# BattleZips/BattleZips-Halo2

Measured on AMD Instinct MI355X. Metric: complete proofs per second (synthesis + create_proof), BoardCircuit, k=14, IPA/Pasta, higher is better.
Workload: dtype u32x8 (255-bit modular integer, Montgomery)

## Files before the change

battlezips-halo2_amd/bzh2/__init__.py:

```python
from __future__ import annotations

import ctypes
import os

import numpy as np

_PKG = os.path.dirname(os.path.abspath(__file__))
_LIB_PATH = os.path.join(os.path.dirname(_PKG), "libbzh2.so")

OK, E_ARG, E_OOM, E_HIP, E_RANGE, E_NOGPU = 0, -1, -2, -3, -4, -5
CURVE_VESTA, CURVE_PALLAS, CURVE_BN254 = 0, 1, 2
FIELD_FP, FIELD_FQ, FIELD_BN254_FR, FIELD_BN254_FQ = 0, 1, 2, 3
FORM_CANONICAL, FORM_MONTGOMERY = 0, 1
MEM_HOST, MEM_DEVICE = 0, 1
T_MSM_DIGITS, T_MSM_ACCUMULATE, T_MSM_REDUCE, T_MSM_FINALIZE, T_NTT, T_COUNT = 0, 1, 2, 3, 4, 8
TIMER_NAMES = {0: "msm_digits", 1: "msm_accumulate", 2: "msm_reduce", 3: "msm_finalize", 4: "ntt"}

CURVE_SCALAR_FIELD = {CURVE_VESTA: FIELD_FP, CURVE_PALLAS: FIELD_FQ, CURVE_BN254: FIELD_BN254_FR}

EXPORTS = [
    "bzh_version", "bzh_strerror", "bzh_device_count", "bzh_ctx_create", "bzh_ctx_create_on_stream",
    "bzh_ctx_destroy", "bzh_ctx_sync", "bzh_last_error", "bzh_ctx_profile", "bzh_ctx_timings", "bzh_ctx_work", "bzh_ctx_msm_additions",
    "bzh_bases_upload", "bzh_bases_precompute", "bzh_bases_free", "bzh_bases_len", "bzh_bases_walk", "bzh_bases_points", "bzh_msm", "bzh_ntt", "bzh_coeff_to_extended",
    "bzh_jacobian_to_affine", "bzh_jacobian_sum", "bzh_affine_compress", "bzh_field_omega",
]


class BzhError(RuntimeError):
    def __init__(self, status: int, where: str, detail: str = ""):
        self.status = status
        super().__init__("%s failed: %s (%d)%s" % (where, _strerror(status), status, (": " + detail) if detail else ""))


_lib = None


def lib_path() -> str:
    return _LIB_PATH
# ... 16 lines not shown
    L.bzh_ctx_create_on_stream.argtypes = [ctypes.c_int, vp, ctypes.POINTER(vp)]
    L.bzh_ctx_destroy.argtypes = [vp]
    L.bzh_ctx_sync.argtypes = [vp]
    L.bzh_last_error.argtypes = [vp]
    L.bzh_last_error.restype = ctypes.c_char_p
    L.bzh_ctx_profile.argtypes = [vp, ctypes.c_int]
    L.bzh_ctx_timings.argtypes = [vp, ctypes.POINTER(ctypes.c_double), u64p]
    L.bzh_bases_upload.argtypes = [vp, ctypes.c_int, vp, ctypes.c_size_t, ctypes.c_int, ctypes.c_int, ctypes.POINTER(vp)]
    L.bzh_bases_precompute.argtypes = [vp, vp, ctypes.c_int]
    L.bzh_bases_free.argtypes = [vp, vp]
    L.bzh_bases_len.argtypes = [vp]
    L.bzh_bases_len.restype = ctypes.c_size_t
    L.bzh_msm.argtypes = [vp, vp, vp, ctypes.c_size_t, ctypes.c_size_t, ctypes.c_int, ctypes.c_int, vp]
    L.bzh_ntt.argtypes = [vp, ctypes.c_int, vp, ctypes.c_uint, ctypes.c_size_t, u64p, u64p, ctypes.c_int, ctypes.c_int,
                          ctypes.c_int]
    L.bzh_jacobian_to_affine.argtypes = [ctypes.c_int, u64p, ctypes.c_size_t, ctypes.c_int, u64p]
    L.bzh_affine_compress.argtypes = [ctypes.c_int, u64p, ctypes.c_size_t, ctypes.c_int, ctypes.POINTER(ctypes.c_uint8)]
    L.bzh_field_omega.argtypes = [ctypes.c_int, ctypes.c_uint, ctypes.c_int, u64p]
    _lib = L
    return L


def _strerror(status: int) -> str:
    try:
        return load().bzh_strerror(status).decode()
    except Exception:
        return "status %d" % status


def device_count() -> int:
# ... 130 lines not shown
            coset_shift: int | None = None, form: int = FORM_CANONICAL) -> np.ndarray:
        a = np.ascontiguousarray(data, dtype=np.uint64).copy()
        shape = a.shape
        if a.ndim == 2:
            a = a.reshape(1, *a.shape)
        batch, n = a.shape[0], a.shape[1]
        log_n = n.bit_length() - 1
        if n == 0 or (1 << log_n) != n:
            raise BzhError(E_ARG, "bzh_ntt", "length must be a power of two")
        w = field_omega(field, log_n, form) if omega is None else int_to_limbs(omega)
        cs = None if coset_shift is None else int_to_limbs(coset_shift)
        rc = load().bzh_ntt(self.handle, field, ctypes.c_void_p(a.ctypes.data), log_n, batch, _u64(w),
                            _u64(cs) if cs is not None else None, int(inverse), form, MEM_HOST)
        self._check(rc, "bzh_ntt")
        return a.reshape(shape)

    def coeff_to_extended(self, field: int, coeffs: np.ndarray, log_ext: int, omega_ext: int | None = None,
                          coset_shift: int | None = None, form: int = FORM_CANONICAL) -> np.ndarray:
        a = np.ascontiguousarray(coeffs, dtype=np.uint64)
        squeeze = a.ndim == 2
        if squeeze:
            a = a.reshape(1, *a.shape)
        batch, n = a.shape[0], a.shape[1]
        log_n = n.bit_length() - 1
        if n != 1 << log_n:
            raise BzhError(E_ARG, "bzh_coeff_to_extended", "length must be a power of two")
        w = field_omega(field, log_ext, form) if omega_ext is None else int_to_limbs(omega_ext)
        sh = None if coset_shift is None else int_to_limbs(coset_shift)
        out = np.zeros((batch, 1 << log_ext, 4), dtype=np.uint64)
        L = load()
# ... 353 lines not shown
```

battlezips-halo2_amd/csrc/capi.hip:

```cpp
#include <cstring>
#include <algorithm>
#include <thread>
#include <new>
#include <vector>

#include "ctx.hpp"
#include "curve.cuh"
#include "host_field.hpp"

namespace bzh {
void ntt_cache_drop(bzh_ctx* ctx);
}

using namespace bzh;

static bool valid_curve(int c) { return c >= 0 && c <= 2; }
static bool valid_field(int f) { return f >= 0 && f <= 3; }
static bool valid_form(int f) { return f == BZH_FORM_CANONICAL || f == BZH_FORM_MONTGOMERY; }
static bool valid_mem(int m) { return m == BZH_MEM_HOST || m == BZH_MEM_DEVICE; }
static unsigned field_two_adicity(int f) {
    unsigned s = 0;
    with_field(f, [&](auto p) {
        s = FieldInfo<decltype(p)>::S;
        return BZH_OK;
// ... 379 lines not shown
            const uint64_t* coset_shift, int inverse, int form, int mem) {
    if (!ctx || !data || !omega || !valid_field(field) || !valid_form(form) || !valid_mem(mem)) return BZH_E_ARG;
    if (log_n > field_two_adicity(field) || log_n > 30) return BZH_E_RANGE;
    if (batch == 0) return BZH_OK;
    std::lock_guard<std::mutex> lk(ctx->mu);
    BZH_HIP_TRY(ctx, hipSetDevice(ctx->device));
    if (mem == BZH_MEM_DEVICE) return ntt_run(ctx, field, (uint32_t*)data, log_n, batch, omega, coset_shift, inverse, form);
    void* stage = nullptr;
    const size_t bytes = (batch << log_n) * 32;
    int rc = ws_ensure(ctx, 3, bytes, &stage);
    if (rc) return rc;
    BZH_HIP_TRY(ctx, hipMemcpyAsync(stage, data, bytes, hipMemcpyHostToDevice, ctx->stream));
    rc = ntt_run(ctx, field, (uint32_t*)stage, log_n, batch, omega, coset_shift, inverse, form);
    if (rc) return rc;
    BZH_HIP_TRY(ctx, hipMemcpyAsync(data, stage, bytes, hipMemcpyDeviceToHost, ctx->stream));
    BZH_HIP_TRY(ctx, hipStreamSynchronize(ctx->stream));
    return BZH_OK;
}

int bzh_coeff_to_extended(bzh_ctx* ctx, int field, const uint64_t* coeffs, unsigned log_n, uint64_t* out, unsigned log_ext,
                          size_t batch, const uint64_t* omega_ext, const uint64_t* coset_shift, int form, int mem) {
    if (!ctx || !coeffs || !out || !omega_ext || !valid_field(field) || !valid_form(form) || !valid_mem(mem)) return BZH_E_ARG;
    if (log_ext > field_two_adicity(field) || log_ext > 30 || log_n > log_ext) return BZH_E_RANGE;
    if (batch == 0) return BZH_OK;
    std::lock_guard<std::mutex> lk(ctx->mu);
    BZH_HIP_TRY(ctx, hipSetDevice(ctx->device));
    const size_t in_elems = batch << log_n, out_elems = batch << log_ext;
    const uint32_t* d_in = (const uint32_t*)coeffs;
    uint32_t* d_out = (uint32_t*)out;
    void* stage = nullptr;
// ... 377 lines not shown
```

battlezips-halo2_amd/csrc/ctx.hpp:

```cpp
#pragma once
#include <hip/hip_runtime.h>
#include <sched.h>

#include <algorithm>
#include <cstdint>
#include <cstdlib>
#include <cstring>
#include <mutex>
#include <string>
#include <vector>

#include "../../include/bzh2.h"

struct bzh_bases {
    int curve = 0;
    size_t n = 0;
    uint32_t* d_xy = nullptr;
    int device = 0;
    int pre_c = 0;
    int pre_nwin = 0;
    size_t row_stride = 0;
    size_t vec_col_stride = 0;
    uint32_t* d_xy29 = nullptr;
};
// ... 213 lines not shown
            hipEvent_t e = ctx->event_pool.back();
            ctx->event_pool.pop_back();
            return e;
        }
        hipEvent_t e = nullptr;
        if (hipEventCreate(&e) != hipSuccess) return nullptr;
        return e;
    }
};

int msm_run(bzh_ctx* ctx, const bzh_bases* bases, const uint32_t* d_scalars, size_t n, size_t batch, int form,
            uint32_t* d_out_xyz);
int msm_run_paired(bzh_ctx* ctx, const bzh_bases* bases, const uint32_t* d_scalars, size_t n_pair, unsigned log_m, size_t batch,
                   int form, uint32_t* d_out_xyz);
int ntt_run(bzh_ctx* ctx, int field, uint32_t* d_data, unsigned log_n, size_t batch, const uint64_t* omega,
            const uint64_t* coset_shift, int inverse, int form);
int ntt_run_padded(bzh_ctx* ctx, int field, uint32_t* d_dst, const uint32_t* d_src, unsigned src_log, unsigned log_n, size_t batch,
                   const uint64_t* omega, const uint64_t* coset_shift, uint32_t* d_out29 = nullptr);
int bases_to_montgomery(bzh_ctx* ctx, int curve, uint32_t* d_xy, size_t n);
int bases_precompute(bzh_ctx* ctx, bzh_bases* bases, int window_bits);
size_t msm_collapse_scratch_bytes(const bzh_bases* srs, size_t cnt, size_t batch, int c_tail);
int msm_collapse_table(bzh_ctx* ctx, const bzh_bases* srs, const uint32_t* d_s, size_t cnt, size_t batch, int c_tail, uint32_t* d_table29, uint32_t* d_table,
                       void* d_scratch, bzh_bases* out);
int field_convert(bzh_ctx* ctx, int field, uint32_t* d, size_t count, int to_mont);
int poly_batch_invert(bzh_ctx* ctx, int field, uint32_t* d, size_t count);
int poly_prefix_product(bzh_ctx* ctx, int field, uint32_t* d, size_t n, size_t batch);
int poly_eval(bzh_ctx* ctx, int field, const uint32_t* coeffs, size_t n, size_t batch, const uint32_t* xs, size_t x_stride,
              uint32_t* out);
int poly_inner_product(bzh_ctx* ctx, int field, const uint32_t* a, const uint32_t* b, size_t n, size_t batch, uint32_t* out);
int poly_fold(bzh_ctx* ctx, int field, const uint32_t* in, size_t half, size_t batch, const uint32_t* u, size_t u_stride,
              uint32_t* out);
int poly_vec_mul(bzh_ctx* ctx, int field, uint32_t* a, const uint32_t* b, size_t count);
int poly_kate_division(bzh_ctx* ctx, int field, const uint32_t* d_c, size_t n, size_t batch, const uint32_t* d_xs, uint32_t* d_q);
int expr_eval(bzh_ctx* ctx, int field, const void* d_prog, int nops, const uint32_t* const* d_cols, const size_t* d_strides,
              const uint32_t* d_consts, size_t const_stride, size_t size, int result_slot, size_t batch, int nslots, uint32_t* d_out);
int expr_eval2(bzh_ctx* ctx, int field, const void* d_prog, int nops, const uint32_t* const* d_cols, const size_t* d_strides,
               const uint32_t* d_consts, size_t const_stride, size_t size, size_t batch, int nlds, uint32_t* d_out);
int random_field(bzh_ctx* ctx, int field, const uint32_t* d_raw, size_t count, uint32_t* d_out);
int ipa_open(bzh_ctx* ctx, const bzh_bases* bases, const uint32_t* d_polys, size_t batch, const uint64_t* blinds,
             const uint64_t* x3s, const uint8_t* rng_bytes, size_t rng_stride, bzh_transcript* const* trs, uint64_t* out_v,
             const uint32_t* d_raw_in = nullptr);
int ipa_verify(bzh_ctx* ctx, const bzh_bases* bases, const uint64_t* commitment_xy, const uint64_t* x3, const uint64_t* v,
               const uint8_t* proof, size_t proof_len, bzh_transcript* tr, const uint64_t* g0_u_w_xy);
int ipa_check_batch(bzh_ctx* ctx, const bzh_bases* bases, size_t batch, size_t nl, const uint64_t* lc_pts, const uint64_t* lc_scal,
                    const uint64_t* cu, int* ok);
bool point_decompress(int curve, const uint8_t* in, uint64_t* xy_canonical);

}
```

battlezips-halo2_amd/csrc/ipa.hip:

```cpp
#include <cstring>
#include <vector>

#include "block.cuh"
#include "ctx.hpp"
#include "curve.cuh"
#include "host_field.hpp"

namespace bzh {

template <class P>
__global__ void __launch_bounds__(256) k_reduce_wide(const uint32_t* __restrict__ in, size_t count, uint32_t* __restrict__ out) {
    const size_t g = blockIdx.x * (size_t)blockDim.x + threadIdx.x;
    if (g >= count) return;
    Fe<P> lo = fe_load<P>(in + g * 16), hi = fe_load<P>(in + g * 16 + 8);
    Fe<P> r2 = fe_r2<P>();
    fe_store(out + g * 8, fe_add(fe_mul(lo, r2), fe_mul(fe_mul(hi, r2), r2)));
}

template <class P>
__global__ void __launch_bounds__(256) k_ipa_s_update(const uint32_t* __restrict__ s, size_t count, const uint32_t* __restrict__ u,
                                                        uint32_t* __restrict__ s_new) {
    const size_t g = blockIdx.x * (size_t)blockDim.x + threadIdx.x;
    if (g >= count) return;
    const Fe<P> v = fe_load<P>(s + g * 8);
    fe_store(s_new + (2 * g) * 8, v);
    fe_store(s_new + (2 * g + 1) * 8, fe_mul(v, fe_load<P>(u)));
}

struct DevBuf {
    void* p = nullptr;
    ~DevBuf() {
// ... 212 lines not shown
    uint32_t* d_vlr = take(B * 2 * 8);
    void* d_out = nullptr;
    BZH_TRY(ws_ensure(ctx, 5, 2 * B * 96, &d_out));

    const unsigned g256 = 256;
    auto grid2 = [&](size_t c) { return dim3((unsigned)((c + g256 - 1) / g256), (unsigned)B); };
    if (B > 65535) return BZH_E_ARG;

    if (d_raw_in) {
        BZH_HIP_TRY(ctx, hipMemcpyAsync(d_raw, d_raw_in, B * nrand * 64, hipMemcpyDeviceToDevice, st));
    } else {
        for (size_t b = 0; b < B; b++)
            BZH_TRY(h2d_small(ctx, d_raw + b * nrand * 16, rng_bytes + b * rng_stride, nrand * 64));
    }
    hipLaunchKernelGGL((k_reduce_wide<SF>), dim3((unsigned)((B * nrand + g256 - 1) / g256)), dim3(g256), 0, st, d_raw, B * nrand,
                       d_rand);
    BZH_HIP_TRY(ctx, hipMemcpy2DAsync(d_spoly, n * 32, d_rand, nrand * 32, n * 32, B, hipMemcpyDeviceToDevice, st));
    std::vector<Fe<SF>> tail(B * ntail);
    for (size_t b = 0; b < B; b++) BZH_TRY(d2h_async(ctx, &tail[b * ntail], d_rand + (b * nrand + n) * 8, ntail * 32));

    std::vector<Fe<SF>> hc(B * kHc, fe_zero<SF>());
    for (size_t b = 0; b < B; b++) hc[b * kHc] = fe_to_mont(fe_from_u64<SF>(x3s + 4 * b));
    auto push_hc = [&]() -> int {
        return h2d_small(ctx, d_hc, hc.data(), B * kHc * 32);
    };
    BZH_TRY(push_hc());
    BZH_TRY(poly_eval(ctx, field, d_spoly, n, B, d_hc, kHc, d_dv));
    hipLaunchKernelGGL((k_sub_at0_batch<SF>), dim3((unsigned)((B + 63) / 64)), dim3(64), 0, st, d_spoly, n, d_dv, B);
    hipLaunchKernelGGL((k_ipa_commit_scalars<SF>), grid2(n + 2), dim3(g256), 0, st, d_spoly, d_rand, n, nrand, d_commit);
    BZH_HIP_TRY(ctx, hipGetLastError());
    BZH_TRY(msm_run(ctx, bases, d_commit, n + 2, B, BZH_FORM_MONTGOMERY, (uint32_t*)d_out));
// ... 298 lines not shown

int ipa_check_batch(bzh_ctx* ctx, const bzh_bases* bases, size_t batch, size_t nl, const uint64_t* lc_pts, const uint64_t* lc_scal,
                    const uint64_t* cu, int* ok) {
    return with_curve(bases->curve, [&](auto c) { return ipa_check_batch_t<decltype(c)>(ctx, bases, batch, nl, lc_pts, lc_scal, cu, ok); });
}

bool point_decompress(int curve, const uint8_t* in, uint64_t* xy_canonical) {
    bool ok = false;
    with_curve(curve, [&](auto c) {
        ok = h_decompress<decltype(c)>(in, xy_canonical);
        return BZH_OK;
    });
    return ok;
}

int random_field(bzh_ctx* ctx, int field, const uint32_t* d_raw, size_t count, uint32_t* d_out) {
    if (!count) return BZH_OK;
    const dim3 grid((unsigned)((count + 255) / 256)), block(256);
    BZH_TRY(with_field(field, [&](auto p) {
        hipLaunchKernelGGL((k_reduce_wide<decltype(p)>), grid, block, 0, ctx->stream, d_raw, count, d_out);
        return BZH_OK;
    }));
    BZH_HIP_TRY(ctx, hipGetLastError());
    return BZH_OK;
}

int ipa_open(bzh_ctx* ctx, const bzh_bases* bases, const uint32_t* d_polys, size_t batch, const uint64_t* blinds,
             const uint64_t* x3s, const uint8_t* rng_bytes, size_t rng_stride, bzh_transcript* const* trs, uint64_t* out_v,
             const uint32_t* d_raw_in) {
    return with_curve(bases->curve, [&](auto c) {
        return ipa_open_t<decltype(c)>(ctx, bases, d_polys, batch, blinds, x3s, rng_bytes, rng_stride, trs, out_v, d_raw_in);
    });
}
int ipa_verify(bzh_ctx* ctx, const bzh_bases* bases, const uint64_t* commitment_xy, const uint64_t* x3, const uint64_t* v,
               const uint8_t* proof, size_t proof_len, bzh_transcript* tr, const uint64_t* g0_u_w_xy) {
// ... 7 lines not shown
```

battlezips-halo2_amd/csrc/ntt.hip:

```cpp
#include <cstdlib>
#include <cstring>
#include <vector>

#include "host_field.hpp"
#include "ntt_common.cuh"

namespace bzh {

template <class P>
void launch_ntt_pass_wave(const NttPassArgs& aa, unsigned tiles, unsigned nb, hipStream_t stream);
extern template void launch_ntt_pass_wave<FpParams>(const NttPassArgs&, unsigned, unsigned, hipStream_t);
extern template void launch_ntt_pass_wave<FqParams>(const NttPassArgs&, unsigned, unsigned, hipStream_t);
extern template void launch_ntt_pass_wave<BnFrParams>(const NttPassArgs&, unsigned, unsigned, hipStream_t);

template <class P, int C, bool FIRST>
__device__ __forceinline__ void stage_group(uint4* tile, const NttPassArgs& g, int s0, int items, int tid) {
    constexpr int E = 1 << C;
    const int r = g.r, logW = g.logW, W = 1 << logW;
    const int ngroups = items >> C;
    const int stride = 1 << (s0 + logW);
    for (int gi = tid; gi < ngroups; gi += kNttThreads) {
        const int col = gi & (W - 1), gg = gi >> logW;
        const int lo = gg & ((1 << s0) - 1), hi = gg >> s0;
        const int base = ((((hi << C) << s0) | lo) << logW) + col;
// ... 263 lines not shown
                wrow = fe_mul(wrow, wa);
            }
            logA += bits[p];
        }
    }
    BZH_HIP_TRY(ctx, hipMalloc((void**)&d.d_tables, words * 4));
    BZH_HIP_TRY(ctx, hipMemcpyAsync(d.d_tables, host.data(), words * 4, hipMemcpyHostToDevice, ctx->stream));
    BZH_HIP_TRY(ctx, hipStreamSynchronize(ctx->stream));
    return BZH_OK;
}

template <class P>
static int ntt_run_t(bzh_ctx* ctx, uint32_t* d_data, unsigned log_n, size_t batch, const uint64_t* omega,
                     const uint64_t* coset_shift, int inverse, int form, const uint32_t* d_src = nullptr, unsigned src_log = 0,
                     uint32_t* d_out29 = nullptr) {
    if (log_n == 0) return d_out29 ? BZH_E_ARG : BZH_OK;
    Fe<P> w, sh = fe_one<P>();
    for (int i = 0; i < 4; i++) {
        w.l[2 * i] = (uint32_t)omega[i];
        w.l[2 * i + 1] = (uint32_t)(omega[i] >> 32);
        if (coset_shift) {
            sh.l[2 * i] = (uint32_t)coset_shift[i];
            sh.l[2 * i + 1] = (uint32_t)(coset_shift[i] >> 32);
        }
    }
    if (form == BZH_FORM_CANONICAL) {
        w = fe_to_mont(w);
        if (coset_shift) sh = fe_to_mont(sh);
    }
    NttCache* cache = cache_for(ctx);
    NttDomain* dom = nullptr;
// ... 13 lines not shown
        memcpy(d.omega, w.l, 32);
        memcpy(d.shift, sh.l, 32);
        int rc = build_domain<P>(ctx, d, w, coset_shift ? &sh : nullptr);
        if (rc) return rc;
        cache->doms.push_back(d);
        dom = &cache->doms.back();
    }
    const size_t total = batch << log_n;
    if (form == BZH_FORM_CANONICAL) {
        int rc = field_convert(ctx, P::id, d_data, total, 1);
        if (rc) return rc;
    }
    int bits[5];
    const int np = plan_passes(log_n, bits);
    int nz = 0;
    if (d_src) {
        if (src_log > log_n || form != BZH_FORM_MONTGOMERY) return BZH_E_ARG;
        nz = (int)(log_n - src_log);
        if ((np < 2 || nz > bits[0] || nz == 0) && !d_data) return BZH_E_ARG;
        if (np < 2 || nz > bits[0] || nz == 0) {
            BZH_HIP_TRY(ctx, hipMemsetAsync(d_data, 0, total * 32, ctx->stream));
            BZH_HIP_TRY(ctx, hipMemcpy2DAsync(d_data, ((size_t)32) << log_n, d_src, ((size_t)32) << src_log, ((size_t)32) << src_log, batch,
                                              hipMemcpyDeviceToDevice, ctx->stream));
            nz = 0;
            d_src = nullptr;
        }
    }
    uint32_t* d_scratch = nullptr;
    if (np >= 2) {
        void* sp = nullptr;
        int rc = ws_ensure(ctx, 0, total * 32, &sp);
        if (rc) return rc;
        d_scratch = (uint32_t*)sp;
    }
    const bool pre = (!inverse && coset_shift);
    const bool post = (inverse != 0);
    int logA = 0;
    for (int p = 0; p < np; p++) {
        NttPassArgs a;
        a.src = (p == 0) ? (nz ? d_src : d_data) : d_scratch;
        a.nz = (p == 0) ? nz : 0;
        a.dst = (p == np - 1) ? d_data : d_scratch;
        a.log_n = log_n;
        a.r = bits[p];
        a.logA = logA;
        a.logB = (int)log_n - logA - bits[p];
        a.last = (p == np - 1);
        int logW = 11 - a.r;
        if (!a.last && logW > a.logB) logW = a.logB;
        if (a.last && logW > logA) logW = logA;
        a.logW = logW;
        a.nprev = p;
        for (int q = 0; q < 4; q++) a.prev_bits[q] = q < p ? bits[q] : 0;
        a.sub_tw = dom->d_tables + dom->off_sub[a.r];
        a.tw_lo = dom->d_tables + dom->off_tw_lo;
// ... 45 lines not shown
                    hipLaunchKernelGGL((k_ntt_pass<P>), grid, blk, 0, ctx->stream, aa);
                }
            }
        }
        BZH_HIP_TRY(ctx, hipGetLastError());
        logA += bits[p];
    }
    if (form == BZH_FORM_CANONICAL) {
        int rc = field_convert(ctx, P::id, d_data, total, 0);
        if (rc) return rc;
    }
    return BZH_OK;
}

template <class P>
__global__ void __launch_bounds__(256) k_field_convert(uint32_t* data, size_t count, int to_mont) {
    size_t gid = blockIdx.x * (size_t)blockDim.x + threadIdx.x;
    if (gid >= count) return;
    Fe<P> v = fe_load<P>(data + gid * 8);
    fe_store(data + gid * 8, to_mont ? fe_to_mont(v) : fe_from_mont(v));
}

int field_convert(bzh_ctx* ctx, int field, uint32_t* d, size_t count, int to_mont) {
    if (!count) return BZH_OK;
    dim3 grid((unsigned)((count + 255) / 256)), block(256);
    BZH_TRY(with_field(field, [&](auto p) {
        hipLaunchKernelGGL((k_field_convert<decltype(p)>), grid, block, 0, ctx->stream, d, count, to_mont);
        return BZH_OK;
    }));
    BZH_HIP_TRY(ctx, hipGetLastError());
    return BZH_OK;
}

int ntt_run(bzh_ctx* ctx, int field, uint32_t* d_data, unsigned log_n, size_t batch, const uint64_t* omega,
            const uint64_t* coset_shift, int inverse, int form) {
    return with_field(field, [&](auto p) { return ntt_run_t<decltype(p)>(ctx, d_data, log_n, batch, omega, coset_shift, inverse, form); });
}

int ntt_run_padded(bzh_ctx* ctx, int field, uint32_t* d_dst, const uint32_t* d_src, unsigned src_log, unsigned log_n, size_t batch,
                   const uint64_t* omega, const uint64_t* coset_shift, uint32_t* d_out29) {
    const int f = BZH_FORM_MONTGOMERY;
    if (d_out29 && field != BZH_FIELD_FP && field != BZH_FIELD_FQ) return BZH_E_ARG;
    return with_field(field, [&](auto p) {
        using P = decltype(p);
        if constexpr (fe29_supported<P>())
            return ntt_run_t<P>(ctx, d_dst, log_n, batch, omega, coset_shift, 0, f, d_src, src_log, d_out29);
        else
            return ntt_run_t<P>(ctx, d_dst, log_n, batch, omega, coset_shift, 0, f, d_src, src_log);
    });
}

// ... 2 lines not shown
```

battlezips-halo2_amd/csrc/prover.hpp:

```cpp
#pragma once
template <class C>
struct Prover {
    using SF = typename CurveInfo<C>::SF;
    using PB = typename C::Base;
    bzh_ctx* ctx;
    bzh_pk& pk;
    const size_t B;
    hipStream_t st;
    const size_t n, en, usable;
    const int field;
    std::vector<bzh_transcript*> T;
    std::vector<const uint8_t*> rng;
    bool seeded = false;
    std::vector<uint32_t> seed_keys;
    uint32_t* d_seed_keys = nullptr;
    uint64_t seed_ctr = 0;
    std::vector<uint64_t> host_ctr;
    std::vector<std::map<int, Fe<SF>>> env;
    Arena& arena;

    Prover(bzh_ctx* c, bzh_pk& p, size_t batch, Arena& ar)
        : ctx(c), pk(p), B(batch), st(c->stream), n(p.n), en(p.en), usable(p.usable), field(p.field), T(batch, nullptr), rng(batch),
          env(batch), arena(ar) {}
    ~Prover() {
// ... 67 lines not shown
    }
    int seed_sync() {
        for (size_t b = 1; b < B; b++)
            if (host_ctr[b] != host_ctr[0]) return BZH_E_ARG;
        seed_ctr += host_ctr[0];
        std::fill(host_ctr.begin(), host_ctr.end(), 0);
        return BZH_OK;
    }
    int seed_rows(size_t count, uint32_t* raw) {
        BZH_TRY(seed_sync());
        hipLaunchKernelGGL(k_chacha20_rows, dim3((unsigned)((count + 255) / 256), (unsigned)B), dim3(256), 0, st, d_seed_keys, seed_ctr, count, raw);
        BZH_HIP_TRY(ctx, hipGetLastError());
        seed_ctr += count;
        return BZH_OK;
    }
    int draw_rows(size_t count, uint32_t* dst) {
        if (!count) return BZH_OK;
        uint32_t* raw = (uint32_t*)arena.alloc(B * count * 64);
        if (!raw) return BZH_E_OOM;
        if (seeded) {
            BZH_TRY(seed_rows(count, raw));
            return random_field(ctx, field, raw, B * count, dst);
        }
        char* stage = nullptr;
        BZH_TRY(h2d_stage(ctx, B * count * 64, &stage));
        for (size_t b = 0; b < B; b++) {
            memcpy(stage + b * count * 64, rng[b], count * 64);
            rng[b] += count * 64;
        }
        BZH_TRY(h2d_commit(ctx, raw, stage, B * count * 64));
        return random_field(ctx, field, raw, B * count, dst);
    }
    Fe<SF> squeeze(size_t b) {
        uint64_t ch[4];
        bzh_transcript_squeeze_challenge(T[b], ch);
        return fe_to_mont(fe_from_u64<SF>(ch));
    }
    void write_scalar(size_t b, const Fe<SF>& v) {
        uint64_t s[4];
        fe_to_u64<SF>(s, fe_from_mont(v));
        bzh_transcript_write_scalar(T[b], s);
    }

    int to_coeff(uint32_t* dst, const uint32_t* src, size_t count) {
        if (!count) return BZH_OK;
        BZH_HIP_TRY(ctx, hipMemcpyAsync(dst, src, count * n * 32, hipMemcpyDeviceToDevice, st));
        return ntt_run(ctx, field, dst, pk.k, count, pk.omega, nullptr, 1, BZH_FORM_MONTGOMERY);
    }
    int to_extended(uint32_t* dst, const uint32_t* polys, size_t count) {
        if (!count) return BZH_OK;
        if (q29) return ntt_run_padded(ctx, field, nullptr, polys, pk.k, pk.ek, count, pk.eomega, pk.zeta, dst);
        return ntt_run_padded(ctx, field, dst, polys, pk.k, pk.ek, count, pk.eomega, pk.zeta);
    }
    int commit(const uint32_t* polys, size_t pitch, size_t count, const std::vector<Fe<SF>>& blinds, std::vector<uint64_t>& xy,
               bool lagrange = false, long shift_row = -1) {
        xy.assign(count * 8, 0);
        if (!count) return BZH_OK;
        ArenaScope scope(arena);
        static const bool no_shift = getenv("BZH_NO_COMMIT_SHIFT") != nullptr;
        const bool wide = lagrange && pk.srs_lagrange->n == n + 3;
        const bool shift = wide && shift_row >= 0 && !no_shift && count <= 65535;
        const size_t cols = wide ? n + 3 : n + 2;
// ... 224 lines not shown
            BZH_TRY(copy2d(inst, n, tmp, inst_rows, inst_rows, B * ni));
        }
        BZH_TRY(to_coeff(inst_polys, inst, B * ni));
        blinds.assign(B * ni, fe_one<SF>());
        if (pk.srs_lagrange) BZH_TRY(commit(inst, n, B * ni, blinds, xy, true));
        else BZH_TRY(commit(inst_polys, n, B * ni, blinds, xy));
        for (size_t b = 0; b < B; b++)
            for (int i = 0; i < ni; i++) bzh_transcript_common_point(T[b], &xy[(b * ni + i) * 8]);
    }

    mark("instance");
    uint32_t* adv = dalloc(B * na * n);
    uint32_t* adv_polys = dalloc(B * na * n);
    if (!adv || !adv_polys) return BZH_E_OOM;
    BZH_HIP_TRY(ctx, hipMemcpyAsync(adv, d_advice_in, B * na * n * 32, hipMemcpyDeviceToDevice, st));
    {
        uint32_t* rows = dalloc(B * na * bf1);
        if (!rows) return BZH_E_OOM;
        BZH_TRY(draw_rows(na * bf1, rows));
        BZH_TRY(copy2d(adv + usable * 8, n, rows, bf1, bf1, B * na));
    }
    std::vector<Fe<SF>> adv_blinds(B * na);
    for (size_t b = 0; b < B; b++)
        for (int i = 0; i < na; i++) adv_blinds[b * na + i] = draw(b);
    BZH_TRY(to_coeff(adv_polys, adv, B * na));
    if (pk.srs_lagrange) BZH_TRY(commit(adv, n, B * na, adv_blinds, xy, true));
    else BZH_TRY(commit(adv_polys, n, B * na, adv_blinds, xy));
    for (size_t b = 0; b < B; b++) {
        for (int i = 0; i < na; i++) bzh_transcript_write_point(T[b], C::id, &xy[(b * na + i) * 8]);
        env[b][SY_THETA] = squeeze(b);
    }
    uint32_t *inst_cosets = nullptr, *adv_cosets = nullptr;
    auto extend_witness = [&]() -> int {
        if (adv_cosets) return BZH_OK;
        inst_cosets = ext_alloc(B * std::max(ni, 1));
        adv_cosets = ext_alloc(B * na);
// ... 23 lines not shown
        Cols reg;
        lag_registry(reg);
        for (int side = 0; side < 2; side++) {
            const std::vector<int>& es = side ? pk.lookups[li].second : pk.lookups[li].first;
            BZH_TRY(run(key(20 + side, li), [&](EPool& ep) {
                std::vector<int> terms;
                for (int e : es) terms.push_back(lower(pk, e, ep, reg, 1));
                return ep.horner(terms, ep.sym(SY_THETA));
            }, reg, n, side ? d.s_c : d.a_c));
        }
        char *ah_c = nullptr, *sh_c = nullptr, *as_c = nullptr;
        BZH_TRY(pin_big_reserve(ctx, 4 * B * n * 32 + ((size_t)3 << 20)));
        BZH_TRY(pin_big_take(ctx, B * n * 32, &ah_c));
        BZH_TRY(pin_big_take(ctx, B * n * 32, &sh_c));
        BZH_TRY(pin_big_take(ctx, B * 2 * n * 32, &as_c));
        uint32_t* canon = dalloc(2 * B * n);
        if (!canon) return BZH_E_OOM;
        BZH_HIP_TRY(ctx, hipMemcpyAsync(canon, d.a_c, B * n * 32, hipMemcpyDeviceToDevice, st));
        BZH_HIP_TRY(ctx, hipMemcpyAsync(canon + B * n * 8, d.s_c, B * n * 32, hipMemcpyDeviceToDevice, st));
        BZH_TRY(field_convert(ctx, field, canon, 2 * B * n, 0));
        BZH_TRY(xfer_launch(ctx, ah_c, canon, B * n * 32, hipMemcpyDeviceToHost));
        BZH_TRY(xfer_launch(ctx, sh_c, canon + B * n * 8, B * n * 32, hipMemcpyDeviceToHost));
        BZH_HIP_TRY(ctx, hipStreamSynchronize(st));
        const uint64_t* ah = (const uint64_t*)ah_c;
        const uint64_t* sh = (const uint64_t*)sh_c;
        mark(" lk:compress+d2h");
        BZH_TRY(extend_witness());
        mark(" lk:extend_witness");
        uint64_t* as = (uint64_t*)as_c;
        for (size_t v = 0; v < 2 * B; v++) memset(as + (v * n + usable) * 4, 0, (n - usable) * 32);
        {
            const size_t nthreads = std::min<size_t>({B, (size_t)host_thread_budget(), (size_t)8});
            std::vector<int> rcs(B, BZH_OK);
            std::vector<std::thread> th;
            auto work = [&](size_t t) {
                for (size_t b = t; b < B; b += nthreads)
                    rcs[b] = bzh_permute_expression_pair(field, &ah[b * n * 4], &sh[b * n * 4], usable, BZH_FORM_CANONICAL,
                                                         as + (b * 2) * n * 4, as + (b * 2 + 1) * n * 4);
            };
            for (size_t t = 1; t < nthreads; t++) th.emplace_back(work, t);
            work(0);
            for (auto& t : th) t.join();
            for (int rc : rcs)
                if (rc) return rc;
        }
        mark(" lk:sort");
        BZH_TRY(h2d_commit(ctx, d.as, as_c, B * 2 * n * 32));
        BZH_TRY(field_convert(ctx, field, d.as, B * 2 * n, 1));
        mark(" lk:h2d");
        {
            uint32_t* rows = dalloc(B * 2 * bf1);
            if (!rows) return BZH_E_OOM;
            BZH_TRY(draw_rows(2 * bf1, rows));
            BZH_TRY(copy2d(d.as + usable * 8, n, rows, bf1, bf1, B * 2));
        }
        d.blinds.resize(B * 2);
        for (size_t b = 0; b < B; b++) {
            d.blinds[2 * b] = draw(b);
            d.blinds[2 * b + 1] = draw(b);
        }
        BZH_TRY(to_coeff(d.polys, d.as, B * 2));
        if (pk.srs_lagrange) BZH_TRY(commit(d.as, n, B * 2, d.blinds, xy, true));
        else BZH_TRY(commit(d.polys, n, B * 2, d.blinds, xy));
        for (size_t b = 0; b < B; b++) {
            bzh_transcript_write_point(T[b], C::id, &xy[(2 * b) * 8]);
            bzh_transcript_write_point(T[b], C::id, &xy[(2 * b + 1) * 8]);
        }
    }
    BZH_TRY(extend_witness());
    for (size_t b = 0; b < B; b++) {
// ... 17 lines not shown
    std::vector<Fe<SF>> z_blinds(B * std::max(nz, 1));
    auto invert_and_scan_all = [&]() -> int {
        mark("  fp:exprs");
        BZH_TRY(poly_batch_invert(ctx, field, den_all, (size_t)nz * B * n));
        mark("  fp:invert");
        BZH_TRY(poly_vec_mul(ctx, field, zt_all, den_all, (size_t)nz * B * n));
        BZH_TRY(poly_prefix_product(ctx, field, zt_all, n, (size_t)nz * B));
        mark("  fp:mul+scan");
        return BZH_OK;
    };
    auto finish_product = [&](int slot, int prev_slot) -> int {
        product_slot(slot);
        if (prev_slot >= 0)
            hipLaunchKernelGGL((k_scale_rows<SF>), dim3((unsigned)((n + 255) / 256), (unsigned)B), dim3(256), 0, st, zt, n,
                               zs + ((size_t)prev_slot * n + usable) * 8, (size_t)nz * n);
        uint32_t* rows = dalloc(B * bf);
        if (!rows) return BZH_E_OOM;
        BZH_TRY(draw_rows(bf, rows));
        BZH_TRY(copy2d(zt + (n - bf) * 8, n, rows, bf, bf, B));
        for (size_t b = 0; b < B; b++) z_blinds[b * nz + slot] = draw(b);
        return copy2d(zs + (size_t)slot * n * 8, (size_t)nz * n, zt, n, n, B);
    };
    auto lag_col = [&](Cols& reg, std::pair<int, int> col) {
        if (col.first == CX_ADVICE) return reg.add(key(K_ADV, col.second), adv + (size_t)col.second * n * 8, (size_t)na * n);
        if (col.first == CX_FIXED) return reg.add(key(K_FIX, col.second), pk.fixed + (size_t)col.second * n * 8, 0);
        return reg.add(key(K_INST, col.second), inst + (size_t)col.second * n * 8, (size_t)ni * n);
    };
    for (int i = 0; i < nsets; i++) {
        const size_t c0 = (size_t)i * pk.chunk_len, c1 = std::min(m, c0 + pk.chunk_len);
        product_slot(i);
        Cols reg;
        for (size_t gj = c0; gj < c1; gj++) {
            lag_col(reg, pk.perm_columns[gj]);
            reg.add(key(K_SIGMA, gj), pk.sigma + gj * n * 8, 0);
// ... 98 lines not shown
    BZH_TRY(ntt_run(ctx, field, h, pk.ek, B, pk.eomega, pk.zeta, 1, BZH_FORM_MONTGOMERY));
    uint32_t* d_flag = (uint32_t*)arena.alloc(256);
    if (!d_flag) return BZH_E_OOM;
    uint32_t h_flag = 0;
    if ((size_t)npieces * n < en) {
        BZH_HIP_TRY(ctx, hipMemsetAsync(d_flag, 0, 4, st));
        const size_t words = (en - (size_t)npieces * n) * 8;
        hipLaunchKernelGGL(k_any_nonzero, dim3((unsigned)((words + 255) / 256), (unsigned)B), dim3(256), 0, st,
                           h + (size_t)npieces * n * 8, words, en * 8, d_flag);
        BZH_TRY(d2h_async(ctx, &h_flag, d_flag, 4));
    }
    std::vector<Fe<SF>> h_blinds(B * npieces);
    for (size_t b = 0; b < B; b++)
        for (int i = 0; i < npieces; i++) h_blinds[b * npieces + i] = draw(b);
    {
        uint32_t* pieces = dalloc(B * npieces * n);
        if (!pieces) return BZH_E_OOM;
        BZH_TRY(copy2d(pieces, (size_t)npieces * n, h, en, (size_t)npieces * n, B));
        BZH_TRY(commit(pieces, n, B * npieces, h_blinds, xy));
    }
    if (h_flag) {
        ctx->last_error = "quotient has higher degree than expected: a witness does not satisfy the constraints";
        return BZH_E_RANGE;
    }
    std::vector<Fe<SF>> xs(B);
    Fe<SF> omega_m;
    {
        uint64_t t[4];
        memcpy(t, pk.omega, 32);
        omega_m = fe_from_u64<SF>(t);
    }
    const Fe<SF> omega_inv = fe_inv(omega_m);
    for (size_t b = 0; b < B; b++) {
        for (int i = 0; i < npieces; i++) bzh_transcript_write_point(T[b], C::id, &xy[(b * npieces + i) * 8]);
// ... 349 lines not shown
```

include/bzh2.h:

```cpp
#ifndef BZH2_H
#define BZH2_H

#include <stddef.h>
#include <stdint.h>

#ifdef __cplusplus
extern "C" {
#endif

typedef struct bzh_ctx bzh_ctx;
typedef struct bzh_bases bzh_bases;
typedef struct bzh_transcript bzh_transcript;

typedef enum {
    BZH_OK = 0,
    BZH_E_ARG = -1,
    BZH_E_OOM = -2,
    BZH_E_HIP = -3,
    BZH_E_RANGE = -4,
    BZH_E_NOGPU = -5,
    BZH_E_VERIFY = -6
} bzh_status;

typedef enum { BZH_CURVE_VESTA = 0, BZH_CURVE_PALLAS = 1, BZH_CURVE_BN254 = 2 } bzh_curve;
// ... 27 lines not shown
int bzh_ctx_work(bzh_ctx* ctx, double* algorithmic_bytes);
int bzh_ctx_msm_additions(bzh_ctx* ctx, uint64_t* additions);

int bzh_bases_upload(bzh_ctx* ctx, int curve, const uint64_t* xy, size_t n, int form, int mem, bzh_bases** out);
int bzh_bases_precompute(bzh_ctx* ctx, bzh_bases* bases, int window_bits);
int bzh_bases_walk(bzh_ctx* ctx, int curve, const uint64_t* g_xy, int form, size_t n, bzh_bases** out);
int bzh_bases_points(bzh_ctx* ctx, const bzh_bases* bases, size_t first, size_t count, uint64_t* out_xy);
int bzh_bases_free(bzh_ctx* ctx, bzh_bases* bases);
size_t bzh_bases_len(const bzh_bases* bases);

int bzh_msm(bzh_ctx* ctx, const bzh_bases* bases, const uint64_t* scalars, size_t n, size_t batch, int form, int mem,
            uint64_t* out_xyz);

int bzh_ntt(bzh_ctx* ctx, int field, uint64_t* data, unsigned log_n, size_t batch, const uint64_t* omega,
            const uint64_t* coset_shift, int inverse, int form, int mem);

int bzh_coeff_to_extended(bzh_ctx* ctx, int field, const uint64_t* coeffs, unsigned log_n, uint64_t* out, unsigned log_ext,
                          size_t batch, const uint64_t* omega_ext, const uint64_t* coset_shift, int form, int mem);

int bzh_field_convert(bzh_ctx* ctx, int field, uint64_t* data, size_t count, int to_montgomery, int mem);
int bzh_random_field(bzh_ctx* ctx, int field, const uint8_t* rng_bytes, size_t count, int form, int mem, uint64_t* out);
int bzh_batch_invert(bzh_ctx* ctx, int field, uint64_t* data, size_t count, int form, int mem);
int bzh_prefix_product(bzh_ctx* ctx, int field, uint64_t* data, size_t n, size_t batch, int form, int mem);
int bzh_eval_polynomial(bzh_ctx* ctx, int field, const uint64_t* coeffs, size_t n, size_t batch, const uint64_t* xs, size_t nx,
                        int form, int mem, uint64_t* out);
int bzh_inner_product(bzh_ctx* ctx, int field, const uint64_t* a, const uint64_t* b, size_t n, size_t batch, int form, int mem,
                      uint64_t* out);
int bzh_fold(bzh_ctx* ctx, int field, const uint64_t* in, size_t half, size_t batch, const uint64_t* u, size_t nu, int form,
             int mem, uint64_t* out);
int bzh_vec_mul(bzh_ctx* ctx, int field, uint64_t* a, const uint64_t* b, size_t count, int form, int mem);
// ... 131 lines not shown
```

Baseline: 722.5.

## Eliminate staging copies in prover via out-of-place NTT, convert, and pitched draws

Adds an out-of-place NTT path so to_coeff reads the source directly instead of first copying into dst. Random blinding rows are reduced straight into pitched destination slots instead of a temp buffer plus copy2d. Field conversion becomes out-of-place, so lookup data converts directly into and out of pinned host buffers with no device staging copies or separate transfers. Quotient pieces are committed in place when the layout already matches. The aim is to cut device-to-device copies and scratch allocations per proof. The tradeoff is that kernels now read and write pinned host memory directly, which may be slower than bulk DMA. A new bzh_ntt_from API is also exposed.

```diff
diff --git a/battlezips-halo2_amd/bzh2/__init__.py b/battlezips-halo2_amd/bzh2/__init__.py
--- a/battlezips-halo2_amd/bzh2/__init__.py
+++ b/battlezips-halo2_amd/bzh2/__init__.py
@@ -21,7 +21,7 @@
 EXPORTS = [
     "bzh_version", "bzh_strerror", "bzh_device_count", "bzh_ctx_create", "bzh_ctx_create_on_stream",
     "bzh_ctx_destroy", "bzh_ctx_sync", "bzh_last_error", "bzh_ctx_profile", "bzh_ctx_timings", "bzh_ctx_work", "bzh_ctx_msm_additions",
-    "bzh_bases_upload", "bzh_bases_precompute", "bzh_bases_free", "bzh_bases_len", "bzh_bases_walk", "bzh_bases_points", "bzh_msm", "bzh_ntt", "bzh_coeff_to_extended",
+    "bzh_bases_upload", "bzh_bases_precompute", "bzh_bases_free", "bzh_bases_len", "bzh_bases_walk", "bzh_bases_points", "bzh_msm", "bzh_ntt", "bzh_ntt_from", "bzh_coeff_to_extended",
     "bzh_jacobian_to_affine", "bzh_jacobian_sum", "bzh_affine_compress", "bzh_field_omega",
 ]
 
@@ -68,6 +68,7 @@
     L.bzh_msm.argtypes = [vp, vp, vp, ctypes.c_size_t, ctypes.c_size_t, ctypes.c_int, ctypes.c_int, vp]
     L.bzh_ntt.argtypes = [vp, ctypes.c_int, vp, ctypes.c_uint, ctypes.c_size_t, u64p, u64p, ctypes.c_int, ctypes.c_int,
                           ctypes.c_int]
+    L.bzh_ntt_from.argtypes = [vp, ctypes.c_int, vp, vp, ctypes.c_uint, ctypes.c_size_t, u64p, u64p, ctypes.c_int, ctypes.c_int]
     L.bzh_jacobian_to_affine.argtypes = [ctypes.c_int, u64p, ctypes.c_size_t, ctypes.c_int, u64p]
     L.bzh_affine_compress.argtypes = [ctypes.c_int, u64p, ctypes.c_size_t, ctypes.c_int, ctypes.POINTER(ctypes.c_uint8)]
     L.bzh_field_omega.argtypes = [ctypes.c_int, ctypes.c_uint, ctypes.c_int, u64p]
@@ -228,6 +229,21 @@
                             _u64(cs) if cs is not None else None, int(inverse), form, MEM_HOST)
         self._check(rc, "bzh_ntt")
         return a.reshape(shape)
+
+    def ntt_from(self, field: int, src: np.ndarray, omega: int | None = None, inverse: bool = False,
+                 coset_shift: int | None = None) -> np.ndarray:
+        a = np.ascontiguousarray(src, dtype=np.uint64)
+        batch, n = a.shape[0], a.shape[1]
+        log_n = n.bit_length() - 1
+        if a.ndim != 3 or n == 0 or (1 << log_n) != n:
+            raise BzhError(E_ARG, "bzh_ntt_from", "want (batch, 2^k, 4)")
+        w = field_omega(field, log_n, FORM_MONTGOMERY) if omega is None else int_to_limbs(omega)
+        cs = None if coset_shift is None else int_to_limbs(coset_shift)
+        out = np.empty_like(a)
+        rc = load().bzh_ntt_from(self.handle, field, ctypes.c_void_p(a.ctypes.data), ctypes.c_void_p(out.ctypes.data), log_n, batch,
+                                 _u64(w), _u64(cs) if cs is not None else None, int(inverse), MEM_HOST)
+        self._check(rc, "bzh_ntt_from")
+        return out
 
     def coeff_to_extended(self, field: int, coeffs: np.ndarray, log_ext: int, omega_ext: int | None = None,
                           coset_shift: int | None = None, form: int = FORM_CANONICAL) -> np.ndarray:
diff --git a/battlezips-halo2_amd/csrc/capi.hip b/battlezips-halo2_amd/csrc/capi.hip
--- a/battlezips-halo2_amd/csrc/capi.hip
+++ b/battlezips-halo2_amd/csrc/capi.hip
@@ -417,6 +417,29 @@
     rc = ntt_run(ctx, field, (uint32_t*)stage, log_n, batch, omega, coset_shift, inverse, form);
     if (rc) return rc;
     BZH_HIP_TRY(ctx, hipMemcpyAsync(data, stage, bytes, hipMemcpyDeviceToHost, ctx->stream));
+    BZH_HIP_TRY(ctx, hipStreamSynchronize(ctx->stream));
+    return BZH_OK;
+}
+
+int bzh_ntt_from(bzh_ctx* ctx, int field, const uint64_t* src, uint64_t* dst, unsigned log_n, size_t batch, const uint64_t* omega,
+                 const uint64_t* coset_shift, int inverse, int mem) {
+    if (!ctx || !src || !dst || src == dst || !omega || !valid_field(field) || !valid_mem(mem)) return BZH_E_ARG;
+    if (log_n > field_two_adicity(field) || log_n > 30) return BZH_E_RANGE;
+    if (batch == 0) return BZH_OK;
+    std::lock_guard<std::mutex> lk(ctx->mu);
+    BZH_HIP_TRY(ctx, hipSetDevice(ctx->device));
+    const int f = BZH_FORM_MONTGOMERY;
+    if (mem == BZH_MEM_DEVICE) return ntt_run(ctx, field, (uint32_t*)dst, log_n, batch, omega, coset_shift, inverse, f, (const uint32_t*)src);
+    void* stage = nullptr;
+    const size_t bytes = (batch << log_n) * 32;
+    int rc = ws_ensure(ctx, 3, 2 * bytes, &stage);
+    if (rc) return rc;
+    uint32_t* d_in = (uint32_t*)stage;
+    uint32_t* d_res = (uint32_t*)((char*)stage + bytes);
+    BZH_HIP_TRY(ctx, hipMemcpyAsync(d_in, src, bytes, hipMemcpyHostToDevice, ctx->stream));
+    rc = ntt_run(ctx, field, d_res, log_n, batch, omega, coset_shift, inverse, f, d_in);
+    if (rc) return rc;
+    BZH_HIP_TRY(ctx, hipMemcpyAsync(dst, d_res, bytes, hipMemcpyDeviceToHost, ctx->stream));
     BZH_HIP_TRY(ctx, hipStreamSynchronize(ctx->stream));
     return BZH_OK;
 }
diff --git a/battlezips-halo2_amd/csrc/ctx.hpp b/battlezips-halo2_amd/csrc/ctx.hpp
--- a/battlezips-halo2_amd/csrc/ctx.hpp
+++ b/battlezips-halo2_amd/csrc/ctx.hpp
@@ -251,7 +251,7 @@
 int msm_run_paired(bzh_ctx* ctx, const bzh_bases* bases, const uint32_t* d_scalars, size_t n_pair, unsigned log_m, size_t batch,
                    int form, uint32_t* d_out_xyz);
 int ntt_run(bzh_ctx* ctx, int field, uint32_t* d_data, unsigned log_n, size_t batch, const uint64_t* omega,
-            const uint64_t* coset_shift, int inverse, int form);
+            const uint64_t* coset_shift, int inverse, int form, const uint32_t* d_src = nullptr);
 int ntt_run_padded(bzh_ctx* ctx, int field, uint32_t* d_dst, const uint32_t* d_src, unsigned src_log, unsigned log_n, size_t batch,
                    const uint64_t* omega, const uint64_t* coset_shift, uint32_t* d_out29 = nullptr);
 int bases_to_montgomery(bzh_ctx* ctx, int curve, uint32_t* d_xy, size_t n);
@@ -260,6 +260,7 @@
 int msm_collapse_table(bzh_ctx* ctx, const bzh_bases* srs, const uint32_t* d_s, size_t cnt, size_t batch, int c_tail, uint32_t* d_table29, uint32_t* d_table,
                        void* d_scratch, bzh_bases* out);
 int field_convert(bzh_ctx* ctx, int field, uint32_t* d, size_t count, int to_mont);
+int field_convert_to(bzh_ctx* ctx, int field, uint32_t* dst, const uint32_t* src, size_t count, int to_mont);
 int poly_batch_invert(bzh_ctx* ctx, int field, uint32_t* d, size_t count);
 int poly_prefix_product(bzh_ctx* ctx, int field, uint32_t* d, size_t n, size_t batch);
 int poly_eval(bzh_ctx* ctx, int field, const uint32_t* coeffs, size_t n, size_t batch, const uint32_t* xs, size_t x_stride,
@@ -273,7 +274,7 @@
               const uint32_t* d_consts, size_t const_stride, size_t size, int result_slot, size_t batch, int nslots, uint32_t* d_out);
 int expr_eval2(bzh_ctx* ctx, int field, const void* d_prog, int nops, const uint32_t* const* d_cols, const size_t* d_strides,
                const uint32_t* d_consts, size_t const_stride, size_t size, size_t batch, int nlds, uint32_t* d_out);
-int random_field(bzh_ctx* ctx, int field, const uint32_t* d_raw, size_t count, uint32_t* d_out);
+int random_field(bzh_ctx* ctx, int field, const uint32_t* d_raw, size_t count, uint32_t* d_out, size_t width = 0, size_t pitch = 0);
 int ipa_open(bzh_ctx* ctx, const bzh_bases* bases, const uint32_t* d_polys, size_t batch, const uint64_t* blinds,
              const uint64_t* x3s, const uint8_t* rng_bytes, size_t rng_stride, bzh_transcript* const* trs, uint64_t* out_v,
              const uint32_t* d_raw_in = nullptr);
diff --git a/battlezips-halo2_amd/csrc/ipa.hip b/battlezips-halo2_amd/csrc/ipa.hip
--- a/battlezips-halo2_amd/csrc/ipa.hip
+++ b/battlezips-halo2_amd/csrc/ipa.hip
@@ -9,12 +9,14 @@
 namespace bzh {
 
 template <class P>
-__global__ void __launch_bounds__(256) k_reduce_wide(const uint32_t* __restrict__ in, size_t count, uint32_t* __restrict__ out) {
+__global__ void __launch_bounds__(256) k_reduce_wide(const uint32_t* __restrict__ in, size_t count, uint32_t* __restrict__ out, size_t width,
+                                                     size_t pitch) {
     const size_t g = blockIdx.x * (size_t)blockDim.x + threadIdx.x;
     if (g >= count) return;
+    const size_t o = width ? (g / width) * pitch + g % width : g;
     Fe<P> lo = fe_load<P>(in + g * 16), hi = fe_load<P>(in + g * 16 + 8);
     Fe<P> r2 = fe_r2<P>();
-    fe_store(out + g * 8, fe_add(fe_mul(lo, r2), fe_mul(fe_mul(hi, r2), r2)));
+    fe_store(out + o * 8, fe_add(fe_mul(lo, r2), fe_mul(fe_mul(hi, r2), r2)));
 }
 
 template <class P>
@@ -257,7 +259,7 @@
             BZH_TRY(h2d_small(ctx, d_raw + b * nrand * 16, rng_bytes + b * rng_stride, nrand * 64));
     }
     hipLaunchKernelGGL((k_reduce_wide<SF>), dim3((unsigned)((B * nrand + g256 - 1) / g256)), dim3(g256), 0, st, d_raw, B * nrand,
-                       d_rand);
+                       d_rand, (size_t)0, (size_t)0);
     BZH_HIP_TRY(ctx, hipMemcpy2DAsync(d_spoly, n * 32, d_rand, nrand * 32, n * 32, B, hipMemcpyDeviceToDevice, st));
     std::vector<Fe<SF>> tail(B * ntail);
     for (size_t b = 0; b < B; b++) BZH_TRY(d2h_async(ctx, &tail[b * ntail], d_rand + (b * nrand + n) * 8, ntail * 32));
@@ -586,11 +588,12 @@
     return ok;
 }
 
-int random_field(bzh_ctx* ctx, int field, const uint32_t* d_raw, size_t count, uint32_t* d_out) {
+int random_field(bzh_ctx* ctx, int field, const uint32_t* d_raw, size_t count, uint32_t* d_out, size_t width, size_t pitch) {
     if (!count) return BZH_OK;
+    if (width && (pitch < width || count % width)) return BZH_E_ARG;
     const dim3 grid((unsigned)((count + 255) / 256)), block(256);
     BZH_TRY(with_field(field, [&](auto p) {
-        hipLaunchKernelGGL((k_reduce_wide<decltype(p)>), grid, block, 0, ctx->stream, d_raw, count, d_out);
+        hipLaunchKernelGGL((k_reduce_wide<decltype(p)>), grid, block, 0, ctx->stream, d_raw, count, d_out, width, pitch);
         return BZH_OK;
     }));
     BZH_HIP_TRY(ctx, hipGetLastError());
diff --git a/battlezips-halo2_amd/csrc/ntt.hip b/battlezips-halo2_amd/csrc/ntt.hip
--- a/battlezips-halo2_amd/csrc/ntt.hip
+++ b/battlezips-halo2_amd/csrc/ntt.hip
@@ -301,7 +301,11 @@
 static int ntt_run_t(bzh_ctx* ctx, uint32_t* d_data, unsigned log_n, size_t batch, const uint64_t* omega,
                      const uint64_t* coset_shift, int inverse, int form, const uint32_t* d_src = nullptr, unsigned src_log = 0,
                      uint32_t* d_out29 = nullptr) {
-    if (log_n == 0) return d_out29 ? BZH_E_ARG : BZH_OK;
+    if (log_n == 0) {
+        if (d_out29) return BZH_E_ARG;
+        if (d_src && d_src != d_data) BZH_HIP_TRY(ctx, hipMemcpyAsync(d_data, d_src, batch * 32, hipMemcpyDeviceToDevice, ctx->stream));
+        return BZH_OK;
+    }
     Fe<P> w, sh = fe_one<P>();
     for (int i = 0; i < 4; i++) {
         w.l[2 * i] = (uint32_t)omega[i];
@@ -345,6 +349,12 @@
     int bits[5];
     const int np = plan_passes(log_n, bits);
     int nz = 0;
+    const uint32_t* d_first = d_data;
+    if (d_src && src_log == log_n) {
+        if (form != BZH_FORM_MONTGOMERY || !d_data || d_src == d_data) return BZH_E_ARG;
+        d_first = d_src;
+        d_src = nullptr;
+    }
     if (d_src) {
         if (src_log > log_n || form != BZH_FORM_MONTGOMERY) return BZH_E_ARG;
         nz = (int)(log_n - src_log);
@@ -369,7 +379,7 @@
     int logA = 0;
     for (int p = 0; p < np; p++) {
         NttPassArgs a;
-        a.src = (p == 0) ? (nz ? d_src : d_data) : d_scratch;
+        a.src = (p == 0) ? (nz ? d_src : d_first) : d_scratch;
         a.nz = (p == 0) ? nz : 0;
         a.dst = (p == np - 1) ? d_data : d_scratch;
         a.log_n = log_n;
@@ -445,27 +455,30 @@
 }
 
 template <class P>
-__global__ void __launch_bounds__(256) k_field_convert(uint32_t* data, size_t count, int to_mont) {
+__global__ void __launch_bounds__(256) k_field_convert(uint32_t* dst, const uint32_t* src, size_t count, int to_mont) {
     size_t gid = blockIdx.x * (size_t)blockDim.x + threadIdx.x;
     if (gid >= count) return;
-    Fe<P> v = fe_load<P>(data + gid * 8);
-    fe_store(data + gid * 8, to_mont ? fe_to_mont(v) : fe_from_mont(v));
-}
-
-int field_convert(bzh_ctx* ctx, int field, uint32_t* d, size_t count, int to_mont) {
+    Fe<P> v = fe_load<P>(src + gid * 8);
+    fe_store(dst + gid * 8, to_mont ? fe_to_mont(v) : fe_from_mont(v));
+}
+
+int field_convert_to(bzh_ctx* ctx, int field, uint32_t* dst, const uint32_t* src, size_t count, int to_mont) {
     if (!count) return BZH_OK;
     dim3 grid((unsigned)((count + 255) / 256)), block(256);
     BZH_TRY(with_field(field, [&](auto p) {
-        hipLaunchKernelGGL((k_field_convert<decltype(p)>), grid, block, 0, ctx->stream, d, count, to_mont);
+        hipLaunchKernelGGL((k_field_convert<decltype(p)>), grid, block, 0, ctx->stream, dst, src, count, to_mont);
         return BZH_OK;
     }));
     BZH_HIP_TRY(ctx, hipGetLastError());
     return BZH_OK;
 }
+int field_convert(bzh_ctx* ctx, int field, uint32_t* d, size_t count, int to_mont) { return field_convert_to(ctx, field, d, d, count, to_mont); }
 
 int ntt_run(bzh_ctx* ctx, int field, uint32_t* d_data, unsigned log_n, size_t batch, const uint64_t* omega,
-            const uint64_t* coset_shift, int inverse, int form) {
-    return with_field(field, [&](auto p) { return ntt_run_t<decltype(p)>(ctx, d_data, log_n, batch, omega, coset_shift, inverse, form); });
+            const uint64_t* coset_shift, int inverse, int form, const uint32_t* d_src) {
+    return with_field(field, [&](auto p) {
+        return ntt_run_t<decltype(p)>(ctx, d_data, log_n, batch, omega, coset_shift, inverse, form, d_src, log_n);
+    });
 }
 
 int ntt_run_padded(bzh_ctx* ctx, int field, uint32_t* d_dst, const uint32_t* d_src, unsigned src_log, unsigned log_n, size_t batch,
diff --git a/battlezips-halo2_amd/csrc/prover.hpp b/battlezips-halo2_amd/csrc/prover.hpp
--- a/battlezips-halo2_amd/csrc/prover.hpp
+++ b/battlezips-halo2_amd/csrc/prover.hpp
@@ -105,13 +105,13 @@
         seed_ctr += count;
         return BZH_OK;
     }
-    int draw_rows(size_t count, uint32_t* dst) {
+    int draw_rows(size_t count, uint32_t* dst, size_t width = 0, size_t pitch = 0) {
         if (!count) return BZH_OK;
         uint32_t* raw = (uint32_t*)arena.alloc(B * count * 64);
         if (!raw) return BZH_E_OOM;
         if (seeded) {
             BZH_TRY(seed_rows(count, raw));
-            return random_field(ctx, field, raw, B * count, dst);
+            return random_field(ctx, field, raw, B * count, dst, width, pitch);
         }
         char* stage = nullptr;
         BZH_TRY(h2d_stage(ctx, B * count * 64, &stage));
@@ -120,7 +120,7 @@
             rng[b] += count * 64;
         }
         BZH_TRY(h2d_commit(ctx, raw, stage, B * count * 64));
-        return random_field(ctx, field, raw, B * count, dst);
+        return random_field(ctx, field, raw, B * count, dst, width, pitch);
     }
     Fe<SF> squeeze(size_t b) {
         uint64_t ch[4];
@@ -135,8 +135,7 @@
 
     int to_coeff(uint32_t* dst, const uint32_t* src, size_t count) {
         if (!count) return BZH_OK;
-        BZH_HIP_TRY(ctx, hipMemcpyAsync(dst, src, count * n * 32, hipMemcpyDeviceToDevice, st));
-        return ntt_run(ctx, field, dst, pk.k, count, pk.omega, nullptr, 1, BZH_FORM_MONTGOMERY);
+        return ntt_run(ctx, field, dst, pk.k, count, pk.omega, nullptr, 1, BZH_FORM_MONTGOMERY, src);
     }
     int to_extended(uint32_t* dst, const uint32_t* polys, size_t count) {
         if (!count) return BZH_OK;
@@ -391,12 +390,7 @@
     uint32_t* adv_polys = dalloc(B * na * n);
     if (!adv || !adv_polys) return BZH_E_OOM;
     BZH_HIP_TRY(ctx, hipMemcpyAsync(adv, d_advice_in, B * na * n * 32, hipMemcpyDeviceToDevice, st));
-    {
-        uint32_t* rows = dalloc(B * na * bf1);
-        if (!rows) return BZH_E_OOM;
-        BZH_TRY(draw_rows(na * bf1, rows));
-        BZH_TRY(copy2d(adv + usable * 8, n, rows, bf1, bf1, B * na));
-    }
+    BZH_TRY(draw_rows(na * bf1, adv + usable * 8, bf1, n));
     std::vector<Fe<SF>> adv_blinds(B * na);
     for (size_t b = 0; b < B; b++)
         for (int i = 0; i < na; i++) adv_blinds[b * na + i] = draw(b);
@@ -450,13 +444,8 @@
         BZH_TRY(pin_big_take(ctx, B * n * 32, &ah_c));
         BZH_TRY(pin_big_take(ctx, B * n * 32, &sh_c));
         BZH_TRY(pin_big_take(ctx, B * 2 * n * 32, &as_c));
-        uint32_t* canon = dalloc(2 * B * n);
-        if (!canon) return BZH_E_OOM;
-        BZH_HIP_TRY(ctx, hipMemcpyAsync(canon, d.a_c, B * n * 32, hipMemcpyDeviceToDevice, st));
-        BZH_HIP_TRY(ctx, hipMemcpyAsync(canon + B * n * 8, d.s_c, B * n * 32, hipMemcpyDeviceToDevice, st));
-        BZH_TRY(field_convert(ctx, field, canon, 2 * B * n, 0));
-        BZH_TRY(xfer_launch(ctx, ah_c, canon, B * n * 32, hipMemcpyDeviceToHost));
-        BZH_TRY(xfer_launch(ctx, sh_c, canon + B * n * 8, B * n * 32, hipMemcpyDeviceToHost));
+        BZH_TRY(field_convert_to(ctx, field, (uint32_t*)ah_c, d.a_c, B * n, 0));
+        BZH_TRY(field_convert_to(ctx, field, (uint32_t*)sh_c, d.s_c, B * n, 0));
         BZH_HIP_TRY(ctx, hipStreamSynchronize(st));
         const uint64_t* ah = (const uint64_t*)ah_c;
         const uint64_t* sh = (const uint64_t*)sh_c;
@@ -481,15 +470,9 @@
                 if (rc) return rc;
         }
         mark(" lk:sort");
-        BZH_TRY(h2d_commit(ctx, d.as, as_c, B * 2 * n * 32));
-        BZH_TRY(field_convert(ctx, field, d.as, B * 2 * n, 1));
+        BZH_TRY(field_convert_to(ctx, field, d.as, (const uint32_t*)as_c, B * 2 * n, 1));
         mark(" lk:h2d");
-        {
-            uint32_t* rows = dalloc(B * 2 * bf1);
-            if (!rows) return BZH_E_OOM;
-            BZH_TRY(draw_rows(2 * bf1, rows));
-            BZH_TRY(copy2d(d.as + usable * 8, n, rows, bf1, bf1, B * 2));
-        }
+        BZH_TRY(draw_rows(2 * bf1, d.as + usable * 8, bf1, n));
         d.blinds.resize(B * 2);
         for (size_t b = 0; b < B; b++) {
             d.blinds[2 * b] = draw(b);
@@ -537,10 +520,7 @@
         if (prev_slot >= 0)
             hipLaunchKernelGGL((k_scale_rows<SF>), dim3((unsigned)((n + 255) / 256), (unsigned)B), dim3(256), 0, st, zt, n,
                                zs + ((size_t)prev_slot * n + usable) * 8, (size_t)nz * n);
-        uint32_t* rows = dalloc(B * bf);
-        if (!rows) return BZH_E_OOM;
-        BZH_TRY(draw_rows(bf, rows));
-        BZH_TRY(copy2d(zt + (n - bf) * 8, n, rows, bf, bf, B));
+        BZH_TRY(draw_rows(bf, zt + (n - bf) * 8, bf, n));
         for (size_t b = 0; b < B; b++) z_blinds[b * nz + slot] = draw(b);
         return copy2d(zs + (size_t)slot * n * 8, (size_t)nz * n, zt, n, n, B);
     };
@@ -669,10 +649,14 @@
     for (size_t b = 0; b < B; b++)
         for (int i = 0; i < npieces; i++) h_blinds[b * npieces + i] = draw(b);
     {
-        uint32_t* pieces = dalloc(B * npieces * n);
-        if (!pieces) return BZH_E_OOM;
-        BZH_TRY(copy2d(pieces, (size_t)npieces * n, h, en, (size_t)npieces * n, B));
-        BZH_TRY(commit(pieces, n, B * npieces, h_blinds, xy));
+        if ((size_t)npieces * n == en) {
+            BZH_TRY(commit(h, n, B * npieces, h_blinds, xy));
+        } else {
+            uint32_t* pieces = dalloc(B * npieces * n);
+            if (!pieces) return BZH_E_OOM;
+            BZH_TRY(copy2d(pieces, (size_t)npieces * n, h, en, (size_t)npieces * n, B));
+            BZH_TRY(commit(pieces, n, B * npieces, h_blinds, xy));
+        }
     }
     if (h_flag) {
         ctx->last_error = "quotient has higher degree than expected: a witness does not satisfy the constraints";
diff --git a/include/bzh2.h b/include/bzh2.h
--- a/include/bzh2.h
+++ b/include/bzh2.h
@@ -65,6 +65,9 @@
 
 int bzh_ntt(bzh_ctx* ctx, int field, uint64_t* data, unsigned log_n, size_t batch, const uint64_t* omega,
             const uint64_t* coset_shift, int inverse, int form, int mem);
+
+int bzh_ntt_from(bzh_ctx* ctx, int field, const uint64_t* src, uint64_t* dst, unsigned log_n, size_t batch, const uint64_t* omega,
+                 const uint64_t* coset_shift, int inverse, int mem);
 
 int bzh_coeff_to_extended(bzh_ctx* ctx, int field, const uint64_t* coeffs, unsigned log_n, uint64_t* out, unsigned log_ext,
                           size_t batch, const uint64_t* omega_ext, const uint64_t* coset_shift, int form, int mem);
```

Result: no change. 725.0 (median of 6 runs) (+0.4%).
